# uc-vision/splat-trainer

Measured on AMD Instinct MI355X. Metric: fwd+bwd Gaussians/s, higher is better.
Workload: dtype f32

## Files before the change

include/gsplat_hip.h:

```cpp
#ifndef GSPLAT_HIP_H
#define GSPLAT_HIP_H

#include <stddef.h>
#include <stdint.h>

#ifdef __cplusplus
extern "C" {
#endif

#define GSR_OK 0
#define GSR_ERR_INVALID_ARGUMENT -1
#define GSR_ERR_WORKSPACE_TOO_SMALL -2
#define GSR_ERR_LAUNCH_FAILED -3
#define GSR_ERR_UNSUPPORTED -4

#define GSR_ROW_FLOATS 16
#define GSR_PARTIAL_FLOATS 12
#define GSR_MAX_FEATURES 16
#define GSR_WIDE_MIN_FEATURES 4

#ifndef GSR_HAVE_RASTER_PARAMS
#define GSR_HAVE_RASTER_PARAMS
typedef struct GsrRasterParamsC {
  float alpha_threshold;
// ... 29 lines not shown
const char* gsr_error_string(int code);

size_t gsr_scan_workspace_bytes(int64_t n);
int gsr_exclusive_scan_u32(const uint32_t* in, uint32_t* out, int64_t n, uint32_t* total_dev, void* workspace,
                           size_t workspace_bytes, void* stream);
int gsr_exclusive_scan_u32_checked(const uint32_t* in, uint32_t* out, int64_t n, uint32_t* total_dev,
                                   uint32_t* overflow_dev, void* workspace, size_t workspace_bytes, void* stream);
size_t gsr_sort_workspace_bytes(int64_t n);
int gsr_sort_pairs_u32(uint32_t* keys_a, uint32_t* vals_a, uint32_t* keys_b, uint32_t* vals_b, int64_t n,
                       int vals_are_iota, int begin_bit, int end_bit, void* workspace, size_t workspace_bytes,
                       const uint32_t* n_dev, void* stream);
int gsr_sort_pairs2_u32(uint32_t* keys_a, uint32_t* vals_a, uint32_t* vals2_a, uint32_t* keys_b, uint32_t* vals_b,
                        uint32_t* vals2_b, int64_t n, int vals_are_iota, int begin_bit, int end_bit, void* workspace,
                        size_t workspace_bytes, const uint32_t* n_dev, void* stream);

size_t gsr_cull_workspace_bytes(int64_t N);
int gsr_frustum_cull(const float* position, int64_t N, const float* T_camera_world, const float* projection,
                     int32_t W, int32_t H, float near_plane, float far_plane, float margin_px,
                     int64_t* indexes_out, uint32_t* count_dev, void* workspace, size_t workspace_bytes, void* stream);

int gsr_project_forward(const float* position, const float* log_scaling, const float* rotation_xyzw,
                        const float* alpha_logit, const int64_t* indexes, int64_t M, const float* T_camera_world,
                        const float* projection, const GsrRasterParamsC* params_host, float* gaussians2d_out,
                        float* depth_out, const uint32_t* count_dev, uint32_t* depth_keys_out, uint32_t depth_key_bias,
                        uint32_t depth_key_max, void* stream);
int gsr_project_backward(const float* position, const float* log_scaling, const float* rotation_xyzw,
                         const float* alpha_logit, const int64_t* indexes, int64_t M, const float* T_camera_world,
                         const float* projection, const GsrRasterParamsC* params_host, const float* dL_dgaussians2d,
                         const float* dL_ddepth, float* d_position, float* d_log_scaling, float* d_rotation,
                         float* d_alpha_logit, int32_t accumulate, void* stream);
// ... 22 lines not shown
                          const int32_t* inverse, int64_t M, int64_t N, int32_t K, const float* camera_pos,
                          const float* jacobian , float* d_sh_features, float* d_positions,
                          void* stream);

int gsr_sh_backward_multi(const float* dL_dcolors_dense, int64_t dense_stride, const float* camera_positions,
                          int64_t camera_stride, int32_t num_cameras, const float* sh_features, const float* positions,
                          int64_t N, int32_t K, float* d_sh_features, float* d_positions, int32_t accumulate,
                          void* stream);

int gsr_project_sh_forward(const float* position, const float* log_scaling, const float* rotation_xyzw,
                           const float* alpha_logit, const float* sh_features, int32_t K, const int64_t* indexes, int64_t M,
                           const float* T_camera_world, const float* projection, const float* camera_pos,
                           const GsrRasterParamsC* params_host, float* rows_out, float* screen_scale_out,
                           float* jacobian_out, const uint32_t* count_dev, uint32_t* depth_keys_out,
                           uint32_t depth_key_bias, uint32_t depth_key_max, void* stream);
int gsr_project_backward_rows(const float* position, const float* log_scaling, const float* rotation_xyzw,
                              const float* alpha_logit, const int64_t* indexes, int64_t M, const int32_t* inverse,
                              int64_t N, const float* T_camera_world, const float* projection,
                              const GsrRasterParamsC* params_host, const float* rows ,
                              const float* grad_rows, const float* dL_dgaussians2d_extra, const float* dL_ddepth,
                              const float* jacobian,
                              float* d_position, float* d_log_scaling, float* d_rotation, float* d_alpha_logit,
                              int32_t mode, float* d_colors_out, float* prune_cost_out, float* split_score_out,
                              float* visibility_out, void* stream);
int gsr_project_backward_rows_camera(const float* position, const float* log_scaling, const float* rotation_xyzw,
                                     const float* alpha_logit, const int64_t* indexes, int64_t M, const int32_t* inverse,
                                     int64_t N, const float* T_camera_world, const float* projection,
                                     const GsrRasterParamsC* params_host, const float* rows, const float* grad_rows,
                                     const float* dL_dgaussians2d_extra, const float* dL_ddepth, const float* jacobian,
                                     float* d_position, float* d_log_scaling, float* d_rotation, float* d_alpha_logit,
                                     int32_t mode, float* d_colors_out, float* prune_cost_out, float* split_score_out,
                                     float* visibility_out, float* camera_partials, float* d_camera, void* stream);

int gsr_depth_key_range(float near_plane, float far_plane, uint32_t* bias_out, uint32_t* max_key_out);
int gsr_depth_keys(const float* depth, int64_t M, uint32_t bias, uint32_t max_key, uint32_t* keys_out, void* stream);
int gsr_pack_rows(const float* gaussians2d, const float* depth, const float* features, int64_t M, int32_t C,
                  const GsrRasterParamsC* params_host, float* rows_out, float* screen_scale_out, void* stream);
int gsr_pack_rows_wide(const float* gaussians2d, const float* depth, const float* features, int64_t M, int32_t C,
                       const GsrRasterParamsC* params_host, float* rows_out, float* feat_rows_out, float* screen_scale_out,
                       void* stream);
int gsr_tile_count(const float* rows, const uint32_t* order, int64_t M, int32_t W, int32_t H,
                   const GsrRasterParamsC* params_host, uint32_t* count_out, uint32_t* tile_hits_out,
                   const uint32_t* M_dev , void* stream);
#define GSR_TILE_COUNT_OFFSETS_MAX 4194304
size_t gsr_tile_count_offsets_workspace_bytes(int64_t M);
int gsr_tile_count_offsets(const float* rows, const uint32_t* order, int64_t M, int32_t W, int32_t H,
                           const GsrRasterParamsC* params_host, uint32_t* count_out, uint32_t* tile_hits_out,
                           const uint32_t* M_dev, uint32_t* offsets_out, uint32_t* total_dev, uint32_t* overflow_flag,
                           void* workspace, size_t workspace_bytes, void* stream);
int gsr_tile_emit(const float* rows, const uint32_t* order, const uint32_t* offsets, const uint32_t* tile_hits, int64_t M,
                  int32_t W, int32_t H, const GsrRasterParamsC* params_host, uint32_t* keys_out, uint32_t* inst2splat_out,
                  int64_t capacity, const uint32_t* M_dev , void* stream);
int gsr_tile_ranges(const uint32_t* sorted_keys, int64_t O, int32_t num_tiles, uint32_t* tile_range,
                    const uint32_t* O_dev , void* stream);

int gsr_segment_thresholds(int32_t seg_pairs_cfg, int32_t heavy_min_cfg, int64_t O, int32_t num_tiles, int32_t needs_grad,
                           int32_t* seg_pairs_out, int32_t* heavy_min_out);
int64_t gsr_segment_capacity(int64_t O, int32_t O_is_bound, int32_t seg_pairs_cfg, int32_t heavy_min_cfg, int32_t num_tiles,
                             int32_t needs_grad);
int64_t gsr_segment_heavy_capacity(int64_t O, int32_t O_is_bound, int32_t seg_pairs_cfg, int32_t heavy_min_cfg,
                                   int32_t num_tiles, int32_t needs_grad);
int gsr_segment_plan(const uint32_t* tile_range, int32_t num_tiles, int32_t seg_pairs_cfg, int32_t heavy_min_cfg,
                     int32_t needs_grad, int64_t O, const uint32_t* O_dev, int64_t capacity, int64_t heavy_capacity,
                     uint32_t* tile_seg_out, uint32_t* seg_desc_out, uint32_t* seg_total_out, uint32_t* tile_order_out,
// ... 299 lines not shown
```

splat-trainer_amd/csrc/binning.hip:

```cpp
#include "gsr_device.h"
#include "../../include/gsplat_hip.h"

namespace {

inline GsrRasterParams to_params(const GsrRasterParamsC* c) {
  GsrRasterParams rp;
  __builtin_memcpy(&rp, c, sizeof(rp));
  return rp;
}
inline unsigned grid_for(int64_t n, int block) { return (unsigned)((n + block - 1) / block); }

__global__ __launch_bounds__(256) void depth_keys_kernel(const float* __restrict__ depth, int64_t M,
                                                         uint32_t* __restrict__ keys, uint32_t bias, uint32_t max_key) {
  const int64_t m = (int64_t)blockIdx.x * blockDim.x + threadIdx.x;
  if (m >= M) return;
  keys[m] = gsr_depth_key(depth[m], bias, max_key);
}

struct TileHits {
  uint32_t origin;
  uint32_t shape;
  uint32_t lo, hi;
};

// ... 35 lines not shown
  uint32_t mine = 0u;
  uint64_t todo = __ballot(large);
  while (todo) {
    const int l = __builtin_ctzll(todo);
    todo &= todo - 1ull;
    const uint32_t n = hits_of_large_extent(
        gsr_bcast(u, l), gsr_bcast(v, l), gsr_bcast(A, l), gsr_bcast(B, l), gsr_bcast(C, l), gsr_bcast(e.qmax, l),
        __builtin_amdgcn_readlane(e.x0, l), __builtin_amdgcn_readlane(e.x1, l), __builtin_amdgcn_readlane(e.y0, l),
        __builtin_amdgcn_readlane(e.y1, l), keys, ranks, (uint32_t)__builtin_amdgcn_readlane((int)o, l), capacity,
        (uint32_t)__builtin_amdgcn_readlane((int)sid, l), tiles_x, lane);
    if (lane == l) mine = n;
  }
  return mine;
}

__device__ __forceinline__ uint32_t tile_count_one(const float* __restrict__ rows, const uint32_t* __restrict__ order,
                                                   int64_t k, bool live, int tiles_x, int tiles_y,
                                                   const GsrRasterParams& rp, TileHits* __restrict__ hits) {
  float2 uv = make_float2(0.f, 0.f), ab = uv, co = uv;
  GsrExtent e;
  e.x0 = e.x1 = e.y0 = e.y1 = 0; e.qmax = 0.f;
  TileHits h;
  h.origin = 0u; h.shape = 0u; h.lo = 0u; h.hi = 0u;
  uint32_t n = 0;
  bool large = false;
  if (live) {
    const int64_t s = order[k];
    const float4* r = reinterpret_cast<const float4*>(rows + GSR_ROW_FLOATS * s);
    const float4 r0 = r[0];
    const float4 r1 = r[1];
    uv = make_float2(r0.x, r0.y); ab = make_float2(r0.z, r0.w); co = make_float2(r1.x, r1.y);
    e = gsr_splat_extent(uv.x, uv.y, ab.x, ab.y, co.x, co.y, rp, tiles_x, tiles_y);
    const int nx = e.x1 - e.x0, ny = e.y1 - e.y0;
    h.origin = (uint32_t)e.x0 | ((uint32_t)e.y0 << 16);
    if (nx > 0 && ny > 0) {
      if (nx * ny <= 32) {
        h.shape = (uint32_t)nx | ((uint32_t)ny << 8);
        uint64_t map = 0ull;
        int t = 0;
        for (int ty = e.y0; ty < e.y1; ++ty)
          for (int tx = e.x0; tx < e.x1; ++tx, ++t) {
            const uint64_t hm = gsr_tile_half_mask(uv.x, uv.y, ab.x, ab.y, co.x, e.qmax, tx, ty);
            map |= hm << (2 * t);
            n += hm ? 1u : 0u;
          }
        h.lo = (uint32_t)map; h.hi = (uint32_t)(map >> 32);
      } else {
        h.shape = 1u << 16;
        large = true;
      }
    }
  }
  const uint32_t nl = wave_large_extents(large, uv.x, uv.y, ab.x, ab.y, co.x, e, nullptr, nullptr, 0u, 0u, 0u, tiles_x,
                                         gsr_lane());
  if (large) n = nl;
  if (live) *reinterpret_cast<uint4*>(hits + k) = make_uint4(h.origin, h.shape, h.lo, h.hi);
  return n;
}

__global__ __launch_bounds__(256) void tile_count_kernel(const float* __restrict__ rows,
                                                         const uint32_t* __restrict__ order, int64_t M, int tiles_x,
                                                         int tiles_y, GsrRasterParams rp, uint32_t* __restrict__ count,
                                                         TileHits* __restrict__ hits,
                                                         const uint32_t* __restrict__ M_dev,
                                                         uint32_t* __restrict__ block_sums) {
  const int64_t k = (int64_t)blockIdx.x * blockDim.x + threadIdx.x;
  const bool live = k < M && !(M_dev && k >= (int64_t)*M_dev);
  uint32_t n = tile_count_one(rows, order, k, live, tiles_x, tiles_y, rp, hits);
  if (k < M) count[k] = n;
  if (block_sums) {
    __shared__ uint32_t s_wave[4];
    n = gsr_wave_sum_u32(n);
    if (gsr_lane() == 0) s_wave[threadIdx.x >> 6] = n;
    __syncthreads();
    if (threadIdx.x == 0) block_sums[blockIdx.x] = (s_wave[0] + s_wave[1]) + (s_wave[2] + s_wave[3]);
  }
}

__global__ __launch_bounds__(256) void offsets_from_sums_kernel(const uint32_t* __restrict__ count, uint32_t n,
                                                                const uint32_t* __restrict__ sums256,
                                                                uint32_t* __restrict__ offsets,
                                                                uint32_t* __restrict__ total_out,
                                                                uint32_t* __restrict__ overflow) {
  __shared__ uint32_t s_wave[4], s_before[4];
  __shared__ float s_f[4];
  const int lane = gsr_lane(), w = (int)(threadIdx.x >> 6);
  const uint32_t base = blockIdx.x * 4096u + threadIdx.x * 16u;
  uint32_t v[16], sum = 0u;
#pragma unroll
  for (int i = 0; i < 16; ++i) {
    v[i] = (base + i < n) ? count[base + i] : 0u;
    sum += v[i];
  }
  uint32_t before = 0u;
  float fbefore = 0.f;
  for (uint32_t j = threadIdx.x; j < blockIdx.x * 16u; j += 256u) {
    const uint32_t b = sums256[j];
    before += b;
    fbefore += (float)b;
  }
  const uint32_t incl = gsr_wave_scan_incl_u32(sum);
  before = gsr_wave_sum_u32(before);
  fbefore = gsr_wave_sum(fbefore + (float)sum);
  if (lane == 63) s_wave[w] = incl;
  if (lane == 0) { s_before[w] = before; s_f[w] = fbefore; }
  __syncthreads();
  uint32_t prefix = (s_before[0] + s_before[1]) + (s_before[2] + s_before[3]), total = 0u;
  uint32_t in_block = 0u;
#pragma unroll
  for (int j = 0; j < 4; ++j) {
    if (j < w) in_block += s_wave[j];
    total += s_wave[j];
  }
  if (threadIdx.x == 0 && (s_f[0] + s_f[1]) + (s_f[2] + s_f[3]) >= 2147000000.f) *overflow = 1u;
  uint32_t run = prefix + in_block + incl - sum;
#pragma unroll
  for (int i = 0; i < 16; ++i) {
    if (base + i < n) offsets[base + i] = run;
    run += v[i];
  }
  if (total_out && blockIdx.x == gridDim.x - 1 && threadIdx.x == 0) *total_out = prefix + total;
}


__global__ __launch_bounds__(256) void tile_emit_kernel(const float* __restrict__ rows,
                                                        const uint32_t* __restrict__ order,
                                                        const uint32_t* __restrict__ offsets,
                                                        const TileHits* __restrict__ hits, int64_t M, int tiles_x,
                                                        int tiles_y, GsrRasterParams rp, uint32_t* __restrict__ keys,
                                                        uint32_t* __restrict__ inst2splat, uint32_t capacity,
                                                        const uint32_t* __restrict__ M_dev) {
  const int64_t k = (int64_t)blockIdx.x * blockDim.x + threadIdx.x;
// ... 289 lines not shown
  depth_keys_kernel<<<grid_for(M, 256), 256, 0, stream>>>(depth, M, keys_out, bias, max_key);
  GSR_CHECK_LAUNCH();
  return GSR_OK;
}

int gsr_tile_count(const float* rows, const uint32_t* order, int64_t M, int32_t W, int32_t H,
                   const GsrRasterParamsC* params_host, uint32_t* count_out, uint32_t* tile_hits_out,
                   const uint32_t* M_dev, void* stream_) {
  hipStream_t stream = reinterpret_cast<hipStream_t>(stream_);
  if (M < 0 || M >= (1ll << 30) || !params_host || W <= 0 || H <= 0) return GSR_ERR_INVALID_ARGUMENT;
  if (params_host->tile_size != 16) return GSR_ERR_UNSUPPORTED;
  if (M == 0) return GSR_OK;
  if (!rows || !order || !count_out || !tile_hits_out) return GSR_ERR_INVALID_ARGUMENT;
  const int tx = (W + 15) / 16, ty = (H + 15) / 16;
  if (tx > 0xFFFF || ty > 0xFFFF) return GSR_ERR_UNSUPPORTED;
  tile_count_kernel<<<grid_for(M, 256), 256, 0, stream>>>(rows, order, M, tx, ty, to_params(params_host), count_out,
                                                         reinterpret_cast<TileHits*>(tile_hits_out), M_dev, nullptr);
  GSR_CHECK_LAUNCH();
  return GSR_OK;
}

size_t gsr_tile_count_offsets_workspace_bytes(int64_t M) {
  return M > 0 ? (size_t)((M + 255) / 256) * sizeof(uint32_t) + 256 : 256;
}

int gsr_tile_count_offsets(const float* rows, const uint32_t* order, int64_t M, int32_t W, int32_t H,
                           const GsrRasterParamsC* params_host, uint32_t* count_out, uint32_t* tile_hits_out,
                           const uint32_t* M_dev, uint32_t* offsets_out, uint32_t* total_dev, uint32_t* overflow_flag,
                           void* workspace, size_t workspace_bytes, void* stream_) {
  hipStream_t stream = reinterpret_cast<hipStream_t>(stream_);
  if (M < 0 || M > GSR_TILE_COUNT_OFFSETS_MAX || !params_host || W <= 0 || H <= 0) return GSR_ERR_INVALID_ARGUMENT;
  if (params_host->tile_size != 16) return GSR_ERR_UNSUPPORTED;
  if (!total_dev || !overflow_flag) return GSR_ERR_INVALID_ARGUMENT;
  if (M == 0) { hipMemsetAsync(total_dev, 0, sizeof(uint32_t), stream); return GSR_OK; }
  if (!rows || !order || !count_out || !tile_hits_out || !offsets_out) return GSR_ERR_INVALID_ARGUMENT;
  if (!workspace || workspace_bytes < gsr_tile_count_offsets_workspace_bytes(M)) return GSR_ERR_WORKSPACE_TOO_SMALL;
  const int tx = (W + 15) / 16, ty = (H + 15) / 16;
  if (tx > 0xFFFF || ty > 0xFFFF) return GSR_ERR_UNSUPPORTED;
  uint32_t* sums = reinterpret_cast<uint32_t*>(workspace);
  tile_count_kernel<<<grid_for(M, 256), 256, 0, stream>>>(rows, order, M, tx, ty, to_params(params_host), count_out,
                                                         reinterpret_cast<TileHits*>(tile_hits_out), M_dev, sums);
  GSR_CHECK_LAUNCH();
  offsets_from_sums_kernel<<<grid_for(M, 4096), 256, 0, stream>>>(count_out, (uint32_t)M, sums, offsets_out, total_dev,
                                                                 overflow_flag);
  GSR_CHECK_LAUNCH();
  return GSR_OK;
}

int gsr_tile_emit(const float* rows, const uint32_t* order, const uint32_t* offsets, const uint32_t* tile_hits, int64_t M,
                  int32_t W, int32_t H, const GsrRasterParamsC* params_host, uint32_t* keys_out, uint32_t* inst2splat_out,
                  int64_t capacity, const uint32_t* M_dev, void* stream_) {
  hipStream_t stream = reinterpret_cast<hipStream_t>(stream_);
  if (M < 0 || M >= (1ll << 30) || !params_host || W <= 0 || H <= 0) return GSR_ERR_INVALID_ARGUMENT;
  if (capacity < 0 || capacity > 0x7FFFFFFFll) return GSR_ERR_INVALID_ARGUMENT;
  if (params_host->tile_size != 16) return GSR_ERR_UNSUPPORTED;
  if (M == 0) return GSR_OK;
  if (!rows || !order || !offsets || !tile_hits || !keys_out || !inst2splat_out) return GSR_ERR_INVALID_ARGUMENT;
  const int tx = (W + 15) / 16, ty = (H + 15) / 16;
  tile_emit_kernel<<<grid_for(M, 256), 256, 0, stream>>>(rows, order, offsets, reinterpret_cast<const TileHits*>(tile_hits),
                                                        M, tx, ty, to_params(params_host), keys_out, inst2splat_out,
                                                        (uint32_t)capacity, M_dev);
// ... 74 lines not shown
```

splat-trainer_amd/csrc/frame.hip:

```cpp
#include <hip/hip_runtime.h>
#include <stdint.h>
#include <string.h>

#include "../../include/gsplat_hip.h"

namespace {

inline int64_t align_up(int64_t x, int64_t a = 256) { return (x + a - 1) / a * a; }

struct Cursor {
  int64_t at = 0;
  int64_t take(int64_t bytes) {
    const int64_t o = at;
    at = align_up(at + (bytes > 0 ? bytes : 1));
    return o;
  }
};

inline int tile_bits_of(int num_tiles) {
  int b = 1;
  while ((1 << b) < num_tiles) ++b;
  return b;
}

// ... 77 lines not shown
  p->out_bytes = out.at;

  Cursor work;
  p->cull_ws_bytes = projected ? 0 : (int64_t)gsr_cull_workspace_bytes(N);
  p->sort_ws_bytes = (int64_t)gsr_sort_workspace_bytes(N);
  p->scan_ws_bytes = (int64_t)gsr_scan_workspace_bytes(N);
  if (N <= GSR_TILE_COUNT_OFFSETS_MAX && (int64_t)gsr_tile_count_offsets_workspace_bytes(N) > p->scan_ws_bytes)
    p->scan_ws_bytes = (int64_t)gsr_tile_count_offsets_workspace_bytes(N);
  p->tsort_ws_bytes = (int64_t)gsr_sort_workspace_bytes(cap);
  p->cull_ws = projected ? -1 : work.take(p->cull_ws_bytes);
  p->sort_ws = work.take(p->sort_ws_bytes);
  p->scan_ws = work.take(p->scan_ws_bytes);
  p->tsort_ws = work.take(p->tsort_ws_bytes);
  p->keys_a = work.take(4 * N);
  p->keys_b = work.take(4 * N);
  p->tile_hits = work.take(16 * N);
  p->tkeys_a = work.take(4 * cap);
  p->tkeys_b = work.take(4 * cap);
  p->work_bytes = work.at;
  return GSR_OK;
}

int gsr_frame_forward(const GsrFrameC* f, const GsrFramePlanC* p, void* out, void* work, GsrFrameResultC* res,
                      uint32_t* counts_host, void* event_counts, void* event_k6_begin, void* event_k6_end,
                      void* stream_) {
  hipStream_t stream = reinterpret_cast<hipStream_t>(stream_);
  if (!f || !p || !out || !work || !res) return GSR_ERR_INVALID_ARGUMENT;
  if (f->N <= 0) return GSR_ERR_INVALID_ARGUMENT;
  const bool projected = f->position == nullptr;
  if (projected) {
    if (!f->gaussians2d || !f->depth || !f->features) return GSR_ERR_INVALID_ARGUMENT;
// ... 8 lines not shown
  uint32_t* M_dev = projected ? nullptr : counts;
  uint32_t* O_dev = counts + 1;
  int rc;
#define GSR_TRY(call)          \
  do {                         \
    rc = (call);               \
    if (rc < 0) return rc;     \
  } while (0)

  if (hipMemsetAsync(at<uint8_t>(out, p->zero_begin), 0, (size_t)p->zero_bytes, stream) != hipSuccess)
    return GSR_ERR_LAUNCH_FAILED;
  float* rows = at<float>(out, p->rows);
  uint32_t key_bias = 0, key_max = 0;
  GSR_TRY(gsr_depth_key_range(f->near_plane, f->far_plane, &key_bias, &key_max));
  uint32_t* keys_a = at<uint32_t>(work, p->keys_a);
  if (projected) {
    if (p->feat_rows >= 0)
      GSR_TRY(gsr_pack_rows_wide(f->gaussians2d, f->depth, f->features, N, f->C, &f->params, rows,
                                 at<float>(out, p->feat_rows), at<float>(out, p->screen_scale), stream_));
    else
      GSR_TRY(gsr_pack_rows(f->gaussians2d, f->depth, f->features, N, f->C, &f->params, rows,
                            at<float>(out, p->screen_scale), stream_));
    if (!f->depth_order) GSR_TRY(gsr_depth_keys(f->depth, N, key_bias, key_max, keys_a, stream_));
  } else {
    int64_t* indexes = at<int64_t>(out, p->indexes);
    GSR_TRY(gsr_frustum_cull(f->position, N, f->T_camera_world, f->projection, f->W, f->H, f->near_plane, f->far_plane,
                             f->params.margin_px, indexes, M_dev, at<uint8_t>(work, p->cull_ws),
                             (size_t)p->cull_ws_bytes, stream_));
    GSR_TRY(gsr_project_sh_forward(f->position, f->log_scaling, f->rotation_xyzw, f->alpha_logit, f->sh_features, f->K,
                                   indexes, N, f->T_camera_world, f->projection, f->camera_pos, &f->params, rows,
                                   at<float>(out, p->screen_scale), at<float>(out, p->jacobian), M_dev,
                                   keys_a, key_bias, key_max, stream_));
  }
  uint32_t* vals_a = at<uint32_t>(out, p->vals_a);
  uint32_t* vals_b = at<uint32_t>(out, p->vals_b);
  const uint32_t* order = f->depth_order;
  res->order = -1;
  if (!order) {
    GSR_TRY(gsr_sort_pairs_u32(keys_a, vals_a, at<uint32_t>(work, p->keys_b), vals_b, N, 1, 0, bit_length(key_max),
                               at<uint8_t>(work, p->sort_ws), (size_t)p->sort_ws_bytes, M_dev, stream_));
    res->order = rc == 1 ? p->vals_b : p->vals_a;
    order = rc == 1 ? vals_b : vals_a;
  }
  uint32_t* count = at<uint32_t>(out, p->count);
  uint32_t* offsets = at<uint32_t>(out, p->offsets);
  uint32_t* hits = at<uint32_t>(work, p->tile_hits);
  if (N <= GSR_TILE_COUNT_OFFSETS_MAX) {
    GSR_TRY(gsr_tile_count_offsets(rows, order, N, f->W, f->H, &f->params, count, hits, M_dev, offsets, O_dev, counts + 2,
                                   at<uint8_t>(work, p->scan_ws), (size_t)p->scan_ws_bytes, stream_));
  } else {
    GSR_TRY(gsr_tile_count(rows, order, N, f->W, f->H, &f->params, count, hits, M_dev, stream_));
    GSR_TRY(gsr_exclusive_scan_u32_checked(count, offsets, N, O_dev, counts + 2, at<uint8_t>(work, p->scan_ws),
                                           (size_t)p->scan_ws_bytes, stream_));
  }
  if (counts_host) {
    if (hipMemcpyAsync(counts_host, counts, 3 * sizeof(uint32_t), hipMemcpyDeviceToHost, stream) != hipSuccess)
      return GSR_ERR_LAUNCH_FAILED;
    if (event_counts && hipEventRecord(reinterpret_cast<hipEvent_t>(event_counts), stream) != hipSuccess)
      return GSR_ERR_LAUNCH_FAILED;
  }
  res->sorted_inst = res->sorted_splat = -1;
  float* image = at<float>(out, p->image);
  if (cap > 0) {
    uint32_t* tkeys_a = at<uint32_t>(work, p->tkeys_a);
// ... 141 lines not shown
```

splat-trainer_amd/csrc/geometry.hip:

```cpp
#include "gsr_device.h"
#include "gsr_dpp_reduce.h"
#include "../../include/gsplat_hip.h"

static_assert(sizeof(GsrRasterParams) == sizeof(GsrRasterParamsC), "raster params layout");

namespace {

constexpr int CULL_ITEMS = 16;
constexpr int CULL_WAVE_SPAN = 64 * CULL_ITEMS;
constexpr int64_t CULL_SELF_PREFIX_MAX_WAVES = 4096;

__global__ __launch_bounds__(256) void cull_count_kernel(const float* __restrict__ pos, int64_t N,
                                                         const float* __restrict__ Tcw, const float* __restrict__ proj,
                                                         int W, int H, float near_p, float far_p, float margin,
                                                         uint32_t* __restrict__ wave_counts, int64_t num_waves) {
  const int64_t wave = (int64_t)blockIdx.x * 4 + (threadIdx.x >> 6);
  if (wave >= num_waves) return;
  const int lane = gsr_lane();
  const GsrCam cam = gsr_load_cam(Tcw, proj);
  const int64_t base = wave * CULL_WAVE_SPAN;
  uint32_t cnt = 0;
#pragma unroll 4
  for (int it = 0; it < CULL_ITEMS; ++it) {
    int64_t i = base + it * 64 + lane;
    bool in = false;
    if (i < N) in = gsr_in_view(cam, pos[3 * i], pos[3 * i + 1], pos[3 * i + 2], W, H, near_p, far_p, margin);
    cnt += (uint32_t)__popcll(__ballot(in));
  }
  if (lane == 0) wave_counts[wave] = cnt;
}

__global__ __launch_bounds__(256) void cull_write_kernel(const float* __restrict__ pos, int64_t N,
                                                         const float* __restrict__ Tcw, const float* __restrict__ proj,
                                                         int W, int H, float near_p, float far_p, float margin,
                                                         const uint32_t* __restrict__ wave_offsets, int64_t num_waves,
                                                         int64_t* __restrict__ indexes,
                                                         uint32_t* __restrict__ count_dev) {
  const int64_t wave = (int64_t)blockIdx.x * 4 + (threadIdx.x >> 6);
  if (wave >= num_waves) return;
  const int lane = gsr_lane();
  const GsrCam cam = gsr_load_cam(Tcw, proj);
  const int64_t base = wave * CULL_WAVE_SPAN;
  uint32_t run;
  if (count_dev) {
    uint32_t before = 0u;
    for (int64_t j = lane; j < wave; j += 64) before += wave_offsets[j];
    run = gsr_wave_sum_u32(before);
    if (wave == num_waves - 1 && lane == 0) *count_dev = run + wave_offsets[wave];
  } else {
    run = wave_offsets[wave];
  }
#pragma unroll 4
  for (int it = 0; it < CULL_ITEMS; ++it) {
    int64_t i = base + it * 64 + lane;
    bool in = false;
    if (i < N) in = gsr_in_view(cam, pos[3 * i], pos[3 * i + 1], pos[3 * i + 2], W, H, near_p, far_p, margin);
    uint64_t m = __ballot(in);
// ... 258 lines not shown
}

template <int K>
struct ShStage {
  static constexpr int ROW = 3 * K;
  static constexpr bool VEC = (ROW % 4) == 0;
  static constexpr int PITCH = ROW | 1;
};

template <int K, bool JAC>
__global__ __launch_bounds__(256) void project_sh_fwd_kernel(
    const float* __restrict__ pos, const float* __restrict__ ls, const float* __restrict__ rot,
    const float* __restrict__ logit, const float* __restrict__ sh, const int64_t* __restrict__ idx, int64_t M,
    const float* __restrict__ Tcw, const float* __restrict__ proj, const float* __restrict__ cam_pos,
    GsrRasterParams rp, float* __restrict__ rows, float* __restrict__ sscale, float* __restrict__ jac,
    const uint32_t* __restrict__ count_dev, uint32_t* __restrict__ depth_keys, uint32_t key_bias, uint32_t key_max) {
  constexpr int ROW = ShStage<K>::ROW, PITCH = ShStage<K>::PITCH;
  constexpr int OUT_FLOATS = 256 * (GSR_ROW_FLOATS + 1 + 9);
  constexpr int STAGE_FLOATS = 256 * PITCH > OUT_FLOATS ? 256 * PITCH : OUT_FLOATS;
  __shared__ float s_rows[STAGE_FLOATS];
  __shared__ int32_t s_idx[256];
  const int64_t count = count_dev ? min(M, (int64_t)*count_dev) : M;
  const int64_t m0 = (int64_t)blockIdx.x * 256;
  if (m0 >= count) return;
  const int tid = (int)threadIdx.x;
  const int64_t m = m0 + tid;
  const bool valid = m < count;
  const int64_t i = valid ? idx[m] : -1;
  s_idx[tid] = (int32_t)i;
  __syncthreads();
  if (ShStage<K>::VEC) {
// ... 38 lines not shown
  constexpr int OP = GSR_ROW_FLOATS + 1;
  float* s_out = s_rows;
  float* s_jac = s_rows + 256 * OP;
  if (valid) {
    float* d = s_out + tid * OP;
    d[0] = o.u; d[1] = o.v; d[2] = o.A; d[3] = o.B; d[4] = o.C; d[5] = o.opacity; d[6] = gsr_qlim(o.opacity, rp);
    const float2 bb = gsr_pixel_bbox(o.u, o.v, o.A, o.B, o.C, o.opacity, rp);
    d[7] = col[0]; d[8] = col[1]; d[9] = col[2]; d[10] = o.depth; d[11] = log2f(o.opacity); d[12] = bb.x; d[13] = bb.y;
    d[14] = 0.f; d[15] = 0.f;
    if (JAC) {
#pragma unroll
      for (int e = 0; e < 9; ++e) s_jac[tid * 9 + e] = J[e];
    }
    *reinterpret_cast<float2*>(sscale + 2 * m) = gsr_screen_scale(o.A, o.B, o.C);
    if (depth_keys) depth_keys[m] = gsr_depth_key(o.depth, key_bias, key_max);
  }
  __syncthreads();
  const int nrows = (int)min((int64_t)256, count - m0);
  float4* out4 = reinterpret_cast<float4*>(rows + (int64_t)GSR_ROW_FLOATS * m0);
#pragma unroll
  for (int it = 0; it < 4; ++it) {
    const int e = it * 256 + tid, row = e >> 2, part = e & 3;
    if (row < nrows) {
      const float* d = s_out + row * OP + 4 * part;
      out4[e] = make_float4(d[0], d[1], d[2], d[3]);
    }
  }
  if (JAC) {
    float* jout = jac + 9 * m0;
    for (int e = tid; e < nrows * 9; e += 256) jout[e] = s_jac[e];
// ... 403 lines not shown
int gsr_abi_version(void) { return GSR_ABI_VERSION; }

const char* gsr_error_string(int code) {
  switch (code) {
    case GSR_OK: return "ok";
    case GSR_ERR_INVALID_ARGUMENT: return "invalid argument";
    case GSR_ERR_WORKSPACE_TOO_SMALL: return "workspace too small";
    case GSR_ERR_LAUNCH_FAILED: return "kernel launch failed";
    case GSR_ERR_UNSUPPORTED: return "unsupported configuration";
    default: return "unknown error";
  }
}

size_t gsr_cull_workspace_bytes(int64_t N) {
  if (N < 0) N = 0;
  int64_t nw = (N + CULL_WAVE_SPAN - 1) / CULL_WAVE_SPAN;
  size_t counts = (((size_t)nw * sizeof(uint32_t) + 255) / 256) * 256;
  return counts + gsr_scan_workspace_bytes(nw) + 256;
}

int gsr_frustum_cull(const float* position, int64_t N, const float* T_camera_world, const float* projection, int32_t W,
                     int32_t H, float near_plane, float far_plane, float margin_px, int64_t* indexes_out,
                     uint32_t* count_dev, void* workspace, size_t workspace_bytes, void* stream_) {
  hipStream_t stream = reinterpret_cast<hipStream_t>(stream_);
  if (N < 0 || N > 0x7FFFFFFFll || !count_dev || !T_camera_world || !projection) return GSR_ERR_INVALID_ARGUMENT;
  if (N == 0) { hipMemsetAsync(count_dev, 0, sizeof(uint32_t), stream); return GSR_OK; }
  if (!position || !indexes_out) return GSR_ERR_INVALID_ARGUMENT;
  if (!workspace || workspace_bytes < gsr_cull_workspace_bytes(N)) return GSR_ERR_WORKSPACE_TOO_SMALL;
  const int64_t nw = (N + CULL_WAVE_SPAN - 1) / CULL_WAVE_SPAN;
  uint32_t* wave_counts = reinterpret_cast<uint32_t*>(workspace);
  size_t counts_bytes = (((size_t)nw * sizeof(uint32_t) + 255) / 256) * 256;
  uint8_t* scan_ws = reinterpret_cast<uint8_t*>(workspace) + counts_bytes;
  const unsigned blocks = grid_for(nw, 4);
  cull_count_kernel<<<blocks, 256, 0, stream>>>(position, N, T_camera_world, projection, W, H, near_plane, far_plane,
                                               margin_px, wave_counts, nw);
  GSR_CHECK_LAUNCH();
  const bool self_prefix = nw <= CULL_SELF_PREFIX_MAX_WAVES;
  if (!self_prefix) {
    int rc = gsr_exclusive_scan_u32(wave_counts, wave_counts, nw, count_dev, scan_ws, workspace_bytes - counts_bytes, stream_);
    if (rc != GSR_OK) return rc;
  }
  cull_write_kernel<<<blocks, 256, 0, stream>>>(position, N, T_camera_world, projection, W, H, near_plane, far_plane,
                                               margin_px, wave_counts, nw, indexes_out, self_prefix ? count_dev : nullptr);
  GSR_CHECK_LAUNCH();
  return GSR_OK;
}

int gsr_project_forward(const float* position, const float* log_scaling, const float* rotation_xyzw,
                        const float* alpha_logit, const int64_t* indexes, int64_t M, const float* T_camera_world,
                        const float* projection, const GsrRasterParamsC* params_host, float* gaussians2d_out,
                        float* depth_out, const uint32_t* count_dev, uint32_t* depth_keys_out, uint32_t depth_key_bias,
                        uint32_t depth_key_max, void* stream_) {
  hipStream_t stream = reinterpret_cast<hipStream_t>(stream_);
  if (M < 0 || !params_host) return GSR_ERR_INVALID_ARGUMENT;
  if (M == 0) return GSR_OK;
  if (!position || !log_scaling || !rotation_xyzw || !alpha_logit || !indexes || !T_camera_world || !projection ||
      !gaussians2d_out || !depth_out)
    return GSR_ERR_INVALID_ARGUMENT;
// ... 74 lines not shown
  if (live && (!dL_dcolors || !camera_partials)) return GSR_ERR_INVALID_ARGUMENT;
  if (live) {
    sh_camera_grad_kernel<<<grid_for(M, 256), 256, 0, stream>>>(dL_dcolors, jacobian, M, camera_partials);
    GSR_CHECK_LAUNCH();
  }
  return gsr_camera_grad_finish(camera_partials, live ? gsr_camera_grad_partial_rows(M) : 0, nullptr, d_camera_pos,
                                stream_);
}

int gsr_project_sh_forward(const float* position, const float* log_scaling, const float* rotation_xyzw,
                           const float* alpha_logit, const float* sh_features, int32_t K, const int64_t* indexes, int64_t M,
                           const float* T_camera_world, const float* projection, const float* camera_pos,
                           const GsrRasterParamsC* params_host, float* rows_out, float* screen_scale_out,
                           float* jacobian_out, const uint32_t* count_dev, uint32_t* depth_keys_out,
                           uint32_t depth_key_bias, uint32_t depth_key_max, void* stream_) {
  hipStream_t stream = reinterpret_cast<hipStream_t>(stream_);
  if (M < 0 || !params_host) return GSR_ERR_INVALID_ARGUMENT;
  if (K != 1 && K != 4 && K != 9 && K != 16) return GSR_ERR_UNSUPPORTED;
  if (M == 0) return GSR_OK;
  if (!position || !log_scaling || !rotation_xyzw || !alpha_logit || !sh_features || !indexes || !T_camera_world ||
      !projection || !camera_pos || !rows_out || !screen_scale_out)
    return GSR_ERR_INVALID_ARGUMENT;
  const unsigned g = grid_for(M, 256);
  const GsrRasterParams rp = to_params(params_host);
#define GSR_LAUNCH_PSF(KK, JJ)                                                                                          \
  project_sh_fwd_kernel<KK, JJ><<<g, 256, 0, stream>>>(position, log_scaling, rotation_xyzw, alpha_logit, sh_features,   \
                                                       indexes, M, T_camera_world, projection, camera_pos, rp, rows_out, \
                                                       screen_scale_out, jacobian_out, count_dev, depth_keys_out,        \
                                                       depth_key_bias, depth_key_max)
  const bool jj = jacobian_out != nullptr;
  switch (K) {
    case 1: if (jj) GSR_LAUNCH_PSF(1, true); else GSR_LAUNCH_PSF(1, false); break;
    case 4: if (jj) GSR_LAUNCH_PSF(4, true); else GSR_LAUNCH_PSF(4, false); break;
    case 9: if (jj) GSR_LAUNCH_PSF(9, true); else GSR_LAUNCH_PSF(9, false); break;
    default: if (jj) GSR_LAUNCH_PSF(16, true); else GSR_LAUNCH_PSF(16, false); break;
  }
#undef GSR_LAUNCH_PSF
  GSR_CHECK_LAUNCH();
  return GSR_OK;
}

int gsr_pack_rows(const float* gaussians2d, const float* depth, const float* features, int64_t M, int32_t C,
                  const GsrRasterParamsC* params_host, float* rows_out, float* screen_scale_out, void* stream_) {
  hipStream_t stream = reinterpret_cast<hipStream_t>(stream_);
// ... 212 lines not shown
```

Baseline: 549.6 million.

## Write compact geometry buffer in projection and use smaller per-thread items for small N

The projection kernel now also writes a compact 6-float geometry record per splat into spare workspace. Tile counting reads that record instead of the 64-byte packed row, which cuts gather bandwidth during binning. Separately, the frustum cull and offsets scan use 4 items per thread instead of 16 when N is under a threshold, which raises block count and parallelism for smaller scenes. The cost is extra writes from projection and a larger workspace.

```diff
diff --git a/include/gsplat_hip.h b/include/gsplat_hip.h
--- a/include/gsplat_hip.h
+++ b/include/gsplat_hip.h
@@ -67,6 +67,9 @@
                         uint32_t* vals2_b, int64_t n, int vals_are_iota, int begin_bit, int end_bit, void* workspace,
                         size_t workspace_bytes, const uint32_t* n_dev, void* stream);
 
+#ifndef GSR_CULL_SMALL_MAX
+#define GSR_CULL_SMALL_MAX 1048576
+#endif
 size_t gsr_cull_workspace_bytes(int64_t N);
 int gsr_frustum_cull(const float* position, int64_t N, const float* T_camera_world, const float* projection,
                      int32_t W, int32_t H, float near_plane, float far_plane, float margin_px,
@@ -119,6 +122,12 @@
                            const GsrRasterParamsC* params_host, float* rows_out, float* screen_scale_out,
                            float* jacobian_out, const uint32_t* count_dev, uint32_t* depth_keys_out,
                            uint32_t depth_key_bias, uint32_t depth_key_max, void* stream);
+int gsr_project_sh_forward_geom(const float* position, const float* log_scaling, const float* rotation_xyzw,
+                                const float* alpha_logit, const float* sh_features, int32_t K, const int64_t* indexes,
+                                int64_t M, const float* T_camera_world, const float* projection, const float* camera_pos,
+                                const GsrRasterParamsC* params_host, float* rows_out, float* screen_scale_out,
+                                float* jacobian_out, const uint32_t* count_dev, uint32_t* depth_keys_out,
+                                uint32_t depth_key_bias, uint32_t depth_key_max, float* geometry_out, void* stream);
 int gsr_project_backward_rows(const float* position, const float* log_scaling, const float* rotation_xyzw,
                               const float* alpha_logit, const int64_t* indexes, int64_t M, const int32_t* inverse,
                               int64_t N, const float* T_camera_world, const float* projection,
@@ -148,11 +157,18 @@
                    const GsrRasterParamsC* params_host, uint32_t* count_out, uint32_t* tile_hits_out,
                    const uint32_t* M_dev , void* stream);
 #define GSR_TILE_COUNT_OFFSETS_MAX 4194304
+#ifndef GSR_OFFSETS_SMALL_MAX
+#define GSR_OFFSETS_SMALL_MAX 1048576
+#endif
 size_t gsr_tile_count_offsets_workspace_bytes(int64_t M);
 int gsr_tile_count_offsets(const float* rows, const uint32_t* order, int64_t M, int32_t W, int32_t H,
                            const GsrRasterParamsC* params_host, uint32_t* count_out, uint32_t* tile_hits_out,
                            const uint32_t* M_dev, uint32_t* offsets_out, uint32_t* total_dev, uint32_t* overflow_flag,
                            void* workspace, size_t workspace_bytes, void* stream);
+int gsr_tile_count_offsets_geom(const float* geometry, const uint32_t* order, int64_t M, int32_t W, int32_t H,
+                                const GsrRasterParamsC* params_host, uint32_t* count_out, uint32_t* tile_hits_out,
+                                const uint32_t* M_dev, uint32_t* offsets_out, uint32_t* total_dev,
+                                uint32_t* overflow_flag, void* workspace, size_t workspace_bytes, void* stream);
 int gsr_tile_emit(const float* rows, const uint32_t* order, const uint32_t* offsets, const uint32_t* tile_hits, int64_t M,
                   int32_t W, int32_t H, const GsrRasterParamsC* params_host, uint32_t* keys_out, uint32_t* inst2splat_out,
                   int64_t capacity, const uint32_t* M_dev , void* stream);
diff --git a/splat-trainer_amd/csrc/binning.hip b/splat-trainer_amd/csrc/binning.hip
--- a/splat-trainer_amd/csrc/binning.hip
+++ b/splat-trainer_amd/csrc/binning.hip
@@ -73,6 +73,7 @@
   return mine;
 }
 
+template <bool GEOM>
 __device__ __forceinline__ uint32_t tile_count_one(const float* __restrict__ rows, const uint32_t* __restrict__ order,
                                                    int64_t k, bool live, int tiles_x, int tiles_y,
                                                    const GsrRasterParams& rp, TileHits* __restrict__ hits) {
@@ -85,10 +86,15 @@
   bool large = false;
   if (live) {
     const int64_t s = order[k];
-    const float4* r = reinterpret_cast<const float4*>(rows + GSR_ROW_FLOATS * s);
-    const float4 r0 = r[0];
-    const float4 r1 = r[1];
-    uv = make_float2(r0.x, r0.y); ab = make_float2(r0.z, r0.w); co = make_float2(r1.x, r1.y);
+    if (GEOM) {
+      const float2* r = reinterpret_cast<const float2*>(rows + 6 * s);
+      uv = r[0]; ab = r[1]; co = r[2];
+    } else {
+      const float4* r = reinterpret_cast<const float4*>(rows + GSR_ROW_FLOATS * s);
+      const float4 r0 = r[0];
+      const float4 r1 = r[1];
+      uv = make_float2(r0.x, r0.y); ab = make_float2(r0.z, r0.w); co = make_float2(r1.x, r1.y);
+    }
     e = gsr_splat_extent(uv.x, uv.y, ab.x, ab.y, co.x, co.y, rp, tiles_x, tiles_y);
     const int nx = e.x1 - e.x0, ny = e.y1 - e.y0;
     h.origin = (uint32_t)e.x0 | ((uint32_t)e.y0 << 16);
@@ -117,6 +123,7 @@
   return n;
 }
 
+template <bool GEOM>
 __global__ __launch_bounds__(256) void tile_count_kernel(const float* __restrict__ rows,
                                                          const uint32_t* __restrict__ order, int64_t M, int tiles_x,
                                                          int tiles_y, GsrRasterParams rp, uint32_t* __restrict__ count,
@@ -125,7 +132,7 @@
                                                          uint32_t* __restrict__ block_sums) {
   const int64_t k = (int64_t)blockIdx.x * blockDim.x + threadIdx.x;
   const bool live = k < M && !(M_dev && k >= (int64_t)*M_dev);
-  uint32_t n = tile_count_one(rows, order, k, live, tiles_x, tiles_y, rp, hits);
+  uint32_t n = tile_count_one<GEOM>(rows, order, k, live, tiles_x, tiles_y, rp, hits);
   if (k < M) count[k] = n;
   if (block_sums) {
     __shared__ uint32_t s_wave[4];
@@ -136,6 +143,7 @@
   }
 }
 
+template <int ITEMS>
 __global__ __launch_bounds__(256) void offsets_from_sums_kernel(const uint32_t* __restrict__ count, uint32_t n,
                                                                 const uint32_t* __restrict__ sums256,
                                                                 uint32_t* __restrict__ offsets,
@@ -144,16 +152,16 @@
   __shared__ uint32_t s_wave[4], s_before[4];
   __shared__ float s_f[4];
   const int lane = gsr_lane(), w = (int)(threadIdx.x >> 6);
-  const uint32_t base = blockIdx.x * 4096u + threadIdx.x * 16u;
-  uint32_t v[16], sum = 0u;
-#pragma unroll
-  for (int i = 0; i < 16; ++i) {
+  const uint32_t base = blockIdx.x * (256u * ITEMS) + threadIdx.x * (uint32_t)ITEMS;
+  uint32_t v[ITEMS], sum = 0u;
+#pragma unroll
+  for (int i = 0; i < ITEMS; ++i) {
     v[i] = (base + i < n) ? count[base + i] : 0u;
     sum += v[i];
   }
   uint32_t before = 0u;
   float fbefore = 0.f;
-  for (uint32_t j = threadIdx.x; j < blockIdx.x * 16u; j += 256u) {
+  for (uint32_t j = threadIdx.x; j < blockIdx.x * (uint32_t)ITEMS; j += 256u) {
     const uint32_t b = sums256[j];
     before += b;
     fbefore += (float)b;
@@ -174,7 +182,7 @@
   if (threadIdx.x == 0 && (s_f[0] + s_f[1]) + (s_f[2] + s_f[3]) >= 2147000000.f) *overflow = 1u;
   uint32_t run = prefix + in_block + incl - sum;
 #pragma unroll
-  for (int i = 0; i < 16; ++i) {
+  for (int i = 0; i < ITEMS; ++i) {
     if (base + i < n) offsets[base + i] = run;
     run += v[i];
   }
@@ -494,8 +502,9 @@
   if (!rows || !order || !count_out || !tile_hits_out) return GSR_ERR_INVALID_ARGUMENT;
   const int tx = (W + 15) / 16, ty = (H + 15) / 16;
   if (tx > 0xFFFF || ty > 0xFFFF) return GSR_ERR_UNSUPPORTED;
-  tile_count_kernel<<<grid_for(M, 256), 256, 0, stream>>>(rows, order, M, tx, ty, to_params(params_host), count_out,
-                                                         reinterpret_cast<TileHits*>(tile_hits_out), M_dev, nullptr);
+  tile_count_kernel<false><<<grid_for(M, 256), 256, 0, stream>>>(rows, order, M, tx, ty, to_params(params_host),
+                                                                count_out, reinterpret_cast<TileHits*>(tile_hits_out),
+                                                                M_dev, nullptr);
   GSR_CHECK_LAUNCH();
   return GSR_OK;
 }
@@ -504,10 +513,10 @@
   return M > 0 ? (size_t)((M + 255) / 256) * sizeof(uint32_t) + 256 : 256;
 }
 
-int gsr_tile_count_offsets(const float* rows, const uint32_t* order, int64_t M, int32_t W, int32_t H,
-                           const GsrRasterParamsC* params_host, uint32_t* count_out, uint32_t* tile_hits_out,
-                           const uint32_t* M_dev, uint32_t* offsets_out, uint32_t* total_dev, uint32_t* overflow_flag,
-                           void* workspace, size_t workspace_bytes, void* stream_) {
+static int tile_count_offsets(bool geom, const float* rows, const uint32_t* order, int64_t M, int32_t W, int32_t H,
+                              const GsrRasterParamsC* params_host, uint32_t* count_out, uint32_t* tile_hits_out,
+                              const uint32_t* M_dev, uint32_t* offsets_out, uint32_t* total_dev, uint32_t* overflow_flag,
+                              void* workspace, size_t workspace_bytes, void* stream_) {
   hipStream_t stream = reinterpret_cast<hipStream_t>(stream_);
   if (M < 0 || M > GSR_TILE_COUNT_OFFSETS_MAX || !params_host || W <= 0 || H <= 0) return GSR_ERR_INVALID_ARGUMENT;
   if (params_host->tile_size != 16) return GSR_ERR_UNSUPPORTED;
@@ -518,13 +527,38 @@
   const int tx = (W + 15) / 16, ty = (H + 15) / 16;
   if (tx > 0xFFFF || ty > 0xFFFF) return GSR_ERR_UNSUPPORTED;
   uint32_t* sums = reinterpret_cast<uint32_t*>(workspace);
-  tile_count_kernel<<<grid_for(M, 256), 256, 0, stream>>>(rows, order, M, tx, ty, to_params(params_host), count_out,
-                                                         reinterpret_cast<TileHits*>(tile_hits_out), M_dev, sums);
-  GSR_CHECK_LAUNCH();
-  offsets_from_sums_kernel<<<grid_for(M, 4096), 256, 0, stream>>>(count_out, (uint32_t)M, sums, offsets_out, total_dev,
-                                                                 overflow_flag);
-  GSR_CHECK_LAUNCH();
-  return GSR_OK;
+  TileHits* hits = reinterpret_cast<TileHits*>(tile_hits_out);
+  if (geom)
+    tile_count_kernel<true><<<grid_for(M, 256), 256, 0, stream>>>(rows, order, M, tx, ty, to_params(params_host), count_out,
+                                                                 hits, M_dev, sums);
+  else
+    tile_count_kernel<false><<<grid_for(M, 256), 256, 0, stream>>>(rows, order, M, tx, ty, to_params(params_host),
+                                                                  count_out, hits, M_dev, sums);
+  GSR_CHECK_LAUNCH();
+  if (M < GSR_OFFSETS_SMALL_MAX)
+    offsets_from_sums_kernel<4><<<grid_for(M, 1024), 256, 0, stream>>>(count_out, (uint32_t)M, sums, offsets_out, total_dev,
+                                                                      overflow_flag);
+  else
+    offsets_from_sums_kernel<16><<<grid_for(M, 4096), 256, 0, stream>>>(count_out, (uint32_t)M, sums, offsets_out,
+                                                                       total_dev, overflow_flag);
+  GSR_CHECK_LAUNCH();
+  return GSR_OK;
+}
+
+int gsr_tile_count_offsets(const float* rows, const uint32_t* order, int64_t M, int32_t W, int32_t H,
+                           const GsrRasterParamsC* params_host, uint32_t* count_out, uint32_t* tile_hits_out,
+                           const uint32_t* M_dev, uint32_t* offsets_out, uint32_t* total_dev, uint32_t* overflow_flag,
+                           void* workspace, size_t workspace_bytes, void* stream_) {
+  return tile_count_offsets(false, rows, order, M, W, H, params_host, count_out, tile_hits_out, M_dev, offsets_out,
+                            total_dev, overflow_flag, workspace, workspace_bytes, stream_);
+}
+
+int gsr_tile_count_offsets_geom(const float* geometry, const uint32_t* order, int64_t M, int32_t W, int32_t H,
+                                const GsrRasterParamsC* params_host, uint32_t* count_out, uint32_t* tile_hits_out,
+                                const uint32_t* M_dev, uint32_t* offsets_out, uint32_t* total_dev,
+                                uint32_t* overflow_flag, void* workspace, size_t workspace_bytes, void* stream_) {
+  return tile_count_offsets(true, geometry, order, M, W, H, params_host, count_out, tile_hits_out, M_dev, offsets_out,
+                            total_dev, overflow_flag, workspace, workspace_bytes, stream_);
 }
 
 int gsr_tile_emit(const float* rows, const uint32_t* order, const uint32_t* offsets, const uint32_t* tile_hits, int64_t M,
diff --git a/splat-trainer_amd/csrc/frame.hip b/splat-trainer_amd/csrc/frame.hip
--- a/splat-trainer_amd/csrc/frame.hip
+++ b/splat-trainer_amd/csrc/frame.hip
@@ -115,7 +115,7 @@
   p->tsort_ws = work.take(p->tsort_ws_bytes);
   p->keys_a = work.take(4 * N);
   p->keys_b = work.take(4 * N);
-  p->tile_hits = work.take(16 * N);
+  p->tile_hits = work.take(align_up(16 * N) + (projected ? 0 : 24 * N));
   p->tkeys_a = work.take(4 * cap);
   p->tkeys_b = work.take(4 * cap);
   p->work_bytes = work.at;
@@ -154,6 +154,7 @@
   uint32_t key_bias = 0, key_max = 0;
   GSR_TRY(gsr_depth_key_range(f->near_plane, f->far_plane, &key_bias, &key_max));
   uint32_t* keys_a = at<uint32_t>(work, p->keys_a);
+  float* geometry = const_cast<float*>(f->gaussians2d);
   if (projected) {
     if (p->feat_rows >= 0)
       GSR_TRY(gsr_pack_rows_wide(f->gaussians2d, f->depth, f->features, N, f->C, &f->params, rows,
@@ -167,10 +168,11 @@
     GSR_TRY(gsr_frustum_cull(f->position, N, f->T_camera_world, f->projection, f->W, f->H, f->near_plane, f->far_plane,
                              f->params.margin_px, indexes, M_dev, at<uint8_t>(work, p->cull_ws),
                              (size_t)p->cull_ws_bytes, stream_));
-    GSR_TRY(gsr_project_sh_forward(f->position, f->log_scaling, f->rotation_xyzw, f->alpha_logit, f->sh_features, f->K,
-                                   indexes, N, f->T_camera_world, f->projection, f->camera_pos, &f->params, rows,
-                                   at<float>(out, p->screen_scale), at<float>(out, p->jacobian), M_dev,
-                                   keys_a, key_bias, key_max, stream_));
+    geometry = at<float>(work, p->tile_hits + align_up(16 * N));
+    GSR_TRY(gsr_project_sh_forward_geom(f->position, f->log_scaling, f->rotation_xyzw, f->alpha_logit, f->sh_features,
+                                        f->K, indexes, N, f->T_camera_world, f->projection, f->camera_pos, &f->params,
+                                        rows, at<float>(out, p->screen_scale), at<float>(out, p->jacobian), M_dev,
+                                        keys_a, key_bias, key_max, geometry, stream_));
   }
   uint32_t* vals_a = at<uint32_t>(out, p->vals_a);
   uint32_t* vals_b = at<uint32_t>(out, p->vals_b);
@@ -186,8 +188,8 @@
   uint32_t* offsets = at<uint32_t>(out, p->offsets);
   uint32_t* hits = at<uint32_t>(work, p->tile_hits);
   if (N <= GSR_TILE_COUNT_OFFSETS_MAX) {
-    GSR_TRY(gsr_tile_count_offsets(rows, order, N, f->W, f->H, &f->params, count, hits, M_dev, offsets, O_dev, counts + 2,
-                                   at<uint8_t>(work, p->scan_ws), (size_t)p->scan_ws_bytes, stream_));
+    GSR_TRY(gsr_tile_count_offsets_geom(geometry, order, N, f->W, f->H, &f->params, count, hits, M_dev, offsets, O_dev,
+                                        counts + 2, at<uint8_t>(work, p->scan_ws), (size_t)p->scan_ws_bytes, stream_));
   } else {
     GSR_TRY(gsr_tile_count(rows, order, N, f->W, f->H, &f->params, count, hits, M_dev, stream_));
     GSR_TRY(gsr_exclusive_scan_u32_checked(count, offsets, N, O_dev, counts + 2, at<uint8_t>(work, p->scan_ws),
diff --git a/splat-trainer_amd/csrc/geometry.hip b/splat-trainer_amd/csrc/geometry.hip
--- a/splat-trainer_amd/csrc/geometry.hip
+++ b/splat-trainer_amd/csrc/geometry.hip
@@ -6,10 +6,10 @@
 
 namespace {
 
-constexpr int CULL_ITEMS = 16;
-constexpr int CULL_WAVE_SPAN = 64 * CULL_ITEMS;
+inline int cull_items_for(int64_t N) { return N < GSR_CULL_SMALL_MAX ? 4 : 16; }
 constexpr int64_t CULL_SELF_PREFIX_MAX_WAVES = 4096;
 
+template <int CULL_ITEMS>
 __global__ __launch_bounds__(256) void cull_count_kernel(const float* __restrict__ pos, int64_t N,
                                                          const float* __restrict__ Tcw, const float* __restrict__ proj,
                                                          int W, int H, float near_p, float far_p, float margin,
@@ -18,7 +18,7 @@
   if (wave >= num_waves) return;
   const int lane = gsr_lane();
   const GsrCam cam = gsr_load_cam(Tcw, proj);
-  const int64_t base = wave * CULL_WAVE_SPAN;
+  const int64_t base = wave * (64 * CULL_ITEMS);
   uint32_t cnt = 0;
 #pragma unroll 4
   for (int it = 0; it < CULL_ITEMS; ++it) {
@@ -30,6 +30,7 @@
   if (lane == 0) wave_counts[wave] = cnt;
 }
 
+template <int CULL_ITEMS>
 __global__ __launch_bounds__(256) void cull_write_kernel(const float* __restrict__ pos, int64_t N,
                                                          const float* __restrict__ Tcw, const float* __restrict__ proj,
                                                          int W, int H, float near_p, float far_p, float margin,
@@ -40,7 +41,7 @@
   if (wave >= num_waves) return;
   const int lane = gsr_lane();
   const GsrCam cam = gsr_load_cam(Tcw, proj);
-  const int64_t base = wave * CULL_WAVE_SPAN;
+  const int64_t base = wave * (64 * CULL_ITEMS);
   uint32_t run;
   if (count_dev) {
     uint32_t before = 0u;
@@ -329,7 +330,8 @@
     const float* __restrict__ logit, const float* __restrict__ sh, const int64_t* __restrict__ idx, int64_t M,
     const float* __restrict__ Tcw, const float* __restrict__ proj, const float* __restrict__ cam_pos,
     GsrRasterParams rp, float* __restrict__ rows, float* __restrict__ sscale, float* __restrict__ jac,
-    const uint32_t* __restrict__ count_dev, uint32_t* __restrict__ depth_keys, uint32_t key_bias, uint32_t key_max) {
+    const uint32_t* __restrict__ count_dev, uint32_t* __restrict__ depth_keys, uint32_t key_bias, uint32_t key_max,
+    float* __restrict__ geom) {
   constexpr int ROW = ShStage<K>::ROW, PITCH = ShStage<K>::PITCH;
   constexpr int OUT_FLOATS = 256 * (GSR_ROW_FLOATS + 1 + 9);
   constexpr int STAGE_FLOATS = 256 * PITCH > OUT_FLOATS ? 256 * PITCH : OUT_FLOATS;
@@ -398,6 +400,10 @@
     }
     *reinterpret_cast<float2*>(sscale + 2 * m) = gsr_screen_scale(o.A, o.B, o.C);
     if (depth_keys) depth_keys[m] = gsr_depth_key(o.depth, key_bias, key_max);
+    if (geom) {
+      float2* gq = reinterpret_cast<float2*>(geom + 6 * m);
+      gq[0] = make_float2(o.u, o.v); gq[1] = make_float2(o.A, o.B); gq[2] = make_float2(o.C, o.opacity);
+    }
   }
   __syncthreads();
   const int nrows = (int)min((int64_t)256, count - m0);
@@ -831,7 +837,8 @@
 
 size_t gsr_cull_workspace_bytes(int64_t N) {
   if (N < 0) N = 0;
-  int64_t nw = (N + CULL_WAVE_SPAN - 1) / CULL_WAVE_SPAN;
+  const int64_t span = 64 * cull_items_for(N);
+  int64_t nw = (N + span - 1) / span;
   size_t counts = (((size_t)nw * sizeof(uint32_t) + 255) / 256) * 256;
   return counts + gsr_scan_workspace_bytes(nw) + 256;
 }
@@ -844,21 +851,31 @@
   if (N == 0) { hipMemsetAsync(count_dev, 0, sizeof(uint32_t), stream); return GSR_OK; }
   if (!position || !indexes_out) return GSR_ERR_INVALID_ARGUMENT;
   if (!workspace || workspace_bytes < gsr_cull_workspace_bytes(N)) return GSR_ERR_WORKSPACE_TOO_SMALL;
-  const int64_t nw = (N + CULL_WAVE_SPAN - 1) / CULL_WAVE_SPAN;
+  const int items = cull_items_for(N);
+  const int64_t nw = (N + 64 * items - 1) / (64 * items);
   uint32_t* wave_counts = reinterpret_cast<uint32_t*>(workspace);
   size_t counts_bytes = (((size_t)nw * sizeof(uint32_t) + 255) / 256) * 256;
   uint8_t* scan_ws = reinterpret_cast<uint8_t*>(workspace) + counts_bytes;
   const unsigned blocks = grid_for(nw, 4);
-  cull_count_kernel<<<blocks, 256, 0, stream>>>(position, N, T_camera_world, projection, W, H, near_plane, far_plane,
-                                               margin_px, wave_counts, nw);
+  if (items == 4)
+    cull_count_kernel<4><<<blocks, 256, 0, stream>>>(position, N, T_camera_world, projection, W, H, near_plane, far_plane,
+                                                    margin_px, wave_counts, nw);
+  else
+    cull_count_kernel<16><<<blocks, 256, 0, stream>>>(position, N, T_camera_world, projection, W, H, near_plane, far_plane,
+                                                     margin_px, wave_counts, nw);
   GSR_CHECK_LAUNCH();
   const bool self_prefix = nw <= CULL_SELF_PREFIX_MAX_WAVES;
   if (!self_prefix) {
     int rc = gsr_exclusive_scan_u32(wave_counts, wave_counts, nw, count_dev, scan_ws, workspace_bytes - counts_bytes, stream_);
     if (rc != GSR_OK) return rc;
   }
-  cull_write_kernel<<<blocks, 256, 0, stream>>>(position, N, T_camera_world, projection, W, H, near_plane, far_plane,
-                                               margin_px, wave_counts, nw, indexes_out, self_prefix ? count_dev : nullptr);
+  uint32_t* cd = self_prefix ? count_dev : nullptr;
+  if (items == 4)
+    cull_write_kernel<4><<<blocks, 256, 0, stream>>>(position, N, T_camera_world, projection, W, H, near_plane, far_plane,
+                                                    margin_px, wave_counts, nw, indexes_out, cd);
+  else
+    cull_write_kernel<16><<<blocks, 256, 0, stream>>>(position, N, T_camera_world, projection, W, H, near_plane, far_plane,
+                                                     margin_px, wave_counts, nw, indexes_out, cd);
   GSR_CHECK_LAUNCH();
   return GSR_OK;
 }
@@ -963,6 +980,18 @@
                            const GsrRasterParamsC* params_host, float* rows_out, float* screen_scale_out,
                            float* jacobian_out, const uint32_t* count_dev, uint32_t* depth_keys_out,
                            uint32_t depth_key_bias, uint32_t depth_key_max, void* stream_) {
+  return gsr_project_sh_forward_geom(position, log_scaling, rotation_xyzw, alpha_logit, sh_features, K, indexes, M,
+                                     T_camera_world, projection, camera_pos, params_host, rows_out, screen_scale_out,
+                                     jacobian_out, count_dev, depth_keys_out, depth_key_bias, depth_key_max, nullptr,
+                                     stream_);
+}
+
+int gsr_project_sh_forward_geom(const float* position, const float* log_scaling, const float* rotation_xyzw,
+                                const float* alpha_logit, const float* sh_features, int32_t K, const int64_t* indexes,
+                                int64_t M, const float* T_camera_world, const float* projection, const float* camera_pos,
+                                const GsrRasterParamsC* params_host, float* rows_out, float* screen_scale_out,
+                                float* jacobian_out, const uint32_t* count_dev, uint32_t* depth_keys_out,
+                                uint32_t depth_key_bias, uint32_t depth_key_max, float* geometry_out, void* stream_) {
   hipStream_t stream = reinterpret_cast<hipStream_t>(stream_);
   if (M < 0 || !params_host) return GSR_ERR_INVALID_ARGUMENT;
   if (K != 1 && K != 4 && K != 9 && K != 16) return GSR_ERR_UNSUPPORTED;
@@ -976,7 +1005,7 @@
   project_sh_fwd_kernel<KK, JJ><<<g, 256, 0, stream>>>(position, log_scaling, rotation_xyzw, alpha_logit, sh_features,   \
                                                        indexes, M, T_camera_world, projection, camera_pos, rp, rows_out, \
                                                        screen_scale_out, jacobian_out, count_dev, depth_keys_out,        \
-                                                       depth_key_bias, depth_key_max)
+                                                       depth_key_bias, depth_key_max, geometry_out)
   const bool jj = jacobian_out != nullptr;
   switch (K) {
     case 1: if (jj) GSR_LAUNCH_PSF(1, true); else GSR_LAUNCH_PSF(1, false); break;
```

Measured after the change: 541.4 million. 1.5% lower.
